# prstrive/SCGaussian

Measured on AMD Instinct MI355X. Metric: train_iters_per_sec, higher is better.
Workload: dtype f32; 1 GPU; S2: 200000 Gaussians, 1008x756, SH degree 3, fwd+bwd per view (BASELINE configs[1] shape: LLFF-fern 3-view training, 200 k Gaussians @ 1008x756); gaussians=200000, width=1008, height=756, sh_degree=3, visible=174771, views=3, parallelism=single, ranks_seen=1, launched_by=single process, grad_bucket_bytes=0, grad_bucket_bytes_per_view=0

## Files before the change

scgaussian_amd/csrc/blend.hip:

```cpp
#include "scg_common.h"
#include "tile_sort.h"

namespace scg {

constexpr float kHalfLog2e = 0.72134752044448170f;
typedef float f32x2 __attribute__((ext_vector_type(2)));
typedef float f32x4 __attribute__((ext_vector_type(4)));

__device__ __forceinline__ bool splat_hits_rect(const float4& a, const float4& b, float x0, float y0) {
    const float dx0 = x0 - a.x, dy0 = y0 - a.y, dx1 = dx0 + 7.0f, dy1 = dy0 + 7.0f;
    const float nx = __builtin_amdgcn_fmed3f(0.0f, dx0, dx1), ny = __builtin_amdgcn_fmed3f(0.0f, dy0, dy1);
    const float cb2 = a.w + a.w;
    const float ya = __builtin_amdgcn_fmed3f(b.w * nx, dy0, dy1);
    const float qa = nx * (a.z * nx + cb2 * ya) + b.x * ya * ya;
    const float xb = __builtin_amdgcn_fmed3f(-a.w * ny * __builtin_amdgcn_rcpf(a.z), dx0, dx1);
    const float qb = ny * (b.x * ny + cb2 * xb) + a.z * xb * xb;
    return !((qa > b.z) && (qb > b.z));
}

__device__ __forceinline__ int quadrant_workgroup(int wg, int n_tiles, const uint2* __restrict__ ranges, int& quad) {
    quad = (wg >> 3) & 3;
    const int per = (n_tiles + 7) >> 3;
    const uint32_t* order = reinterpret_cast<const uint32_t*>(ranges) + 2 * (size_t)n_tiles;
    return (int)order[(wg & 7) * per + (wg >> 5)];
}

__device__ __forceinline__ void wave_sync() {
    __builtin_amdgcn_fence(__ATOMIC_ACQ_REL, "wavefront");
    __builtin_amdgcn_wave_barrier();
}

typedef const uint32_t __attribute__((address_space(3))) * LdsIds;
template <class IdList>
__device__ __forceinline__ void forward_walk(float4* s_rec, const FrameDev& f, int tile, int quad, int lane, uint2 range,
                                             IdList list,
                                             const float4* __restrict__ splats, float* __restrict__ out_color,
                                             float* __restrict__ out_depth, float* __restrict__ out_alpha,
                                             float* __restrict__ final_T, uint32_t* __restrict__ n_contrib) {
    const int tile_x = tile % f.gx, tile_y = tile / f.gx;
    const int qx0 = tile_x * kTile + (quad & 1) * 8, qy0 = tile_y * kTile + (quad >> 1) * 8;
    const int px = qx0 + (lane & 7), py = qy0 + (lane >> 3);
    const bool inside = (px < f.W) && (py < f.H);
    const float pxf = (float)px, pyf = (float)py;

    const int n = (int)(range.y - range.x);
    float T = inside ? 1.0f : -1.0f;
    int bgi0 = __builtin_amdgcn_readfirstlane(__builtin_bit_cast(int, f.bg[0]));
    int bgi1 = __builtin_amdgcn_readfirstlane(__builtin_bit_cast(int, f.bg[1]));
    int bgi2 = __builtin_amdgcn_readfirstlane(__builtin_bit_cast(int, f.bg[2]));
    asm volatile("" : "+s"(bgi0), "+s"(bgi1), "+s"(bgi2));
    f32x2 Crg = {0.f, 0.f}, Cbz = {0.f, 0.f};
    uint32_t last = 0;
    int n_blended = 0;
#ifndef SCG_FWD_TRIP_CXX
    const uint32_t lds_base = (uint32_t)reinterpret_cast<uintptr_t>(s_rec);
    const uint64_t exec_all = __builtin_amdgcn_read_exec();
#endif

    uint32_t id_next = 0;
    float4 ra, rb, rc;
    if (n > 0) {
        const uint32_t id0 = list[min(lane, n - 1)];
        id_next = list[min(kWave + lane, n - 1)];
        ra = splats[3 * (size_t)id0 + 0]; rb = splats[3 * (size_t)id0 + 1]; rc = splats[3 * (size_t)id0 + 2];
    }

    for (int base = 0; base < n; base += kWave) {
        if (__all(T < 0.0f)) break;
        const bool hit = (base + lane < n) && splat_hits_rect(ra, rb, (float)qx0, (float)qy0);
        if (hit) {
            *reinterpret_cast<float2*>(&s_rec[2 * kWave + lane]) = make_float2(ra.x, ra.y);
            s_rec[kWave + lane] = make_float4(kHalfLog2e * ra.z, 2.0f * kHalfLog2e * ra.w, kHalfLog2e * rb.x, rb.y);
            s_rec[lane] = rc;
        }
        uint64_t m = __ballot(hit);
        if (base + kWave < n) {
            ra = splats[3 * (size_t)id_next + 0]; rb = splats[3 * (size_t)id_next + 1];
            rc = splats[3 * (size_t)id_next + 2];
            id_next = list[min(base + 2 * kWave + lane, n - 1)];
        }
        wave_sync();

        n_blended += __builtin_popcountll(m);
#ifdef SCG_FWD_TRIP_CXX
        while (m) {
            const int j = __builtin_ctzll(m);
            asm("s_bitset0_b64 %0, %1" : "+s"(m) : "s"(j));
            const float2 c = *reinterpret_cast<const float2*>(&s_rec[2 * kWave + j]);
            const float4 q = s_rec[kWave + j];
            const float dx = c.x - pxf, dy = c.y - pyf;
            const float u = __builtin_fmaf(q.y, dy, q.x * dx);
            const float t = __builtin_fmaf(u, dx, (q.z * dy) * dy);
            const float alpha = fminf(kAlphaMax, q.w * __builtin_amdgcn_exp2f(-t));
            const float wgt = T * alpha;
            const float test_T = __builtin_fmaf(-T, alpha, T);
            if ((t >= 0.0f) && (alpha >= kAlphaMin)) {
                const bool contributes = test_T >= kTEps;
                const float T_prev = T;
                T = contributes ? test_T : -fabsf(T_prev);
                if (contributes) {
                    const float4 col = s_rec[j];
                    const f32x2 ww = {wgt, wgt};
                    Crg = __builtin_elementwise_fma((f32x2){col.x, col.y}, ww, Crg);
                    Cbz = __builtin_elementwise_fma((f32x2){col.z, col.w}, ww, Cbz);
                    last = (uint32_t)(base + j + 1);
                }
            }
        }
#else
        int last_j = -1;
        while (m) {
            const int j = __builtin_ctzll(m);
            asm("s_bitset0_b64 %0, %1" : "+s"(m) : "s"(j));
            asm volatile(
                "v_lshl_add_u32 v63, %[j], 4, %[lds]\n\t"
                "ds_read_b64 v[48:49], v63 offset:2048\n\t"
                "ds_read_b128 v[52:55], v63 offset:1024\n\t"
                "s_waitcnt lgkmcnt(1)\n\t"
                "v_sub_f32_e32 v48, v48, %[px]\n\t"
                "v_sub_f32_e32 v49, v49, %[py]\n\t"
                "s_waitcnt lgkmcnt(0)\n\t"
                "v_mul_f32_e32 v58, v52, v48\n\t"
                "v_mul_f32_e32 v59, v54, v49\n\t"
                "v_fmac_f32_e32 v58, v53, v49\n\t"
                "v_mul_f32_e32 v60, v59, v49\n\t"
                "v_fmac_f32_e32 v60, v58, v48\n\t"
                "v_exp_f32_e64 v56, -v60\n\t"
                "v_cmpx_le_f32_e32 vcc, 0, v60\n\t"
                "v_mul_f32_e32 v56, v55, v56\n\t"
                "v_min_f32_e32 v56, 0x3f7d70a4, v56\n\t"
                "v_cmpx_le_f32_e32 vcc, %[amin], v56\n\t"
                "v_fma_f32 v57, -%[T], v56, %[T]\n\t"
                "v_mul_f32_e32 v56, %[T], v56\n\t"
                "v_or_b32_e32 %[T], 0x80000000, %[T]\n\t"
                "v_cmpx_le_f32_e32 vcc, %[eps], v57\n\t"
                "v_mov_b32_e32 %[T], v57\n\t"
                "ds_read_b128 v[44:47], v63\n\t"
                "v_mov_b32_e32 %[lj], %[j]\n\t"
                "s_waitcnt lgkmcnt(0)\n\t"
                "v_pk_fma_f32 %[crg], v[44:45], v[56:57], %[crg] op_sel_hi:[1,0,1]\n\t"
                "v_pk_fma_f32 %[cbz], v[46:47], v[56:57], %[cbz] op_sel_hi:[1,0,1]\n\t"
                "s_mov_b64 exec, %[all]"
                : [T] "+v"(T), [crg] "+v"(Crg), [cbz] "+v"(Cbz), [lj] "+v"(last_j)
                : [j] "s"(j), [lds] "v"(lds_base), [px] "v"(pxf), [py] "v"(pyf), [amin] "s"(kAlphaMin), [eps] "s"(kTEps),
                  [all] "s"(exec_all)
                : "memory", "vcc", "v44", "v45", "v46", "v47", "v48", "v49", "v52", "v53", "v54", "v55", "v56", "v57", "v58",
                  "v59", "v60", "v63");
        }
        if (last_j >= 0) last = (uint32_t)(base + last_j + 1);
#endif
        wave_sync();
    }

    if (f.cost_out && lane == 0) atomicMax(f.cost_out + tile, (uint32_t)n_blended);
    if (inside) {
        T = fabsf(T);
        const size_t pix = (size_t)py * f.W + px;
        const size_t hw = (size_t)f.H * f.W;
        out_color[pix] = Crg[0] + T * __builtin_bit_cast(float, bgi0);
        out_color[hw + pix] = Crg[1] + T * __builtin_bit_cast(float, bgi1);
        out_color[2 * hw + pix] = Cbz[0] + T * __builtin_bit_cast(float, bgi2);
        out_depth[pix] = Cbz[1];
        out_alpha[pix] = 1.0f - T;
        if (final_T) final_T[pix] = T;
        if (n_contrib) n_contrib[pix] = last;
    }
}


__global__ __launch_bounds__(kWave) void blend_forward_kernel(FrameDev f, const uint2* __restrict__ ranges,
                                                              const uint32_t* __restrict__ point_list,
                                                              const float4* __restrict__ splats,
                                                              float* __restrict__ out_color,
                                                              float* __restrict__ out_depth,
                                                              float* __restrict__ out_alpha,
                                                              float* __restrict__ final_T,
                                                              uint32_t* __restrict__ n_contrib,
                                                              float4* __restrict__ zero_fill, uint32_t zero_vec) {
    __shared__ float4 s_rec[3 * kWave];
    if (zero_fill) {
        for (uint32_t i = blockIdx.x * kWave + threadIdx.x; i < zero_vec; i += gridDim.x * kWave)
            zero_fill[i] = make_float4(0.f, 0.f, 0.f, 0.f);
    }

    const int n_tiles = f.gx * f.gy;
    int quad;
    const int tile = quadrant_workgroup(blockIdx.x, n_tiles, ranges, quad);
    if (tile >= n_tiles) return;
    const uint2 range = ranges[tile];
    forward_walk(s_rec, f, tile, quad, (int)threadIdx.x, range, point_list + range.x, splats, out_color, out_depth, out_alpha,
                 final_T, n_contrib);
}

template <int NW>
__device__ __forceinline__ void fused_long_list_fallback(unsigned char* smem, const uint32_t* __restrict__ depth_keys,
                                                      uint32_t* __restrict__ list, int n, uint64_t* __restrict__ keys,
                                                      uint64_t* __restrict__ keys2) {
    if (!sort_long_list<NW * kWave, kFusedLongBuckets, 2>(smem, depth_keys, list, n, keys, keys2)) {
        __syncthreads();
        for (int i = threadIdx.x; i < n; i += NW * kWave) {
            const uint32_t id = list[i];
            keys[i] = ((uint64_t)depth_keys[id] << 32) | (uint64_t)id;
        }
        __syncthreads();
        bitonic_sort_asc(keys, n, true);
        __syncthreads();
        for (int i = threadIdx.x; i < n; i += NW * kWave) list[i] = (uint32_t)keys[i];
    }
}

template <int MAX_N, int CNT, int WPE, int NW = 4>
__global__ __launch_bounds__(NW * kWave) __attribute__((amdgpu_waves_per_eu(WPE, WPE))) void tile_blend_forward_kernel(
    FrameDev f, const uint2* __restrict__ ranges, uint32_t* __restrict__ point_list,
    const uint32_t* __restrict__ depth_keys, int id_bits, const float4* __restrict__ splats,
    float* __restrict__ out_color, float* __restrict__ out_depth, float* __restrict__ out_alpha,
    float* __restrict__ final_T, uint32_t* __restrict__ n_contrib, float4* __restrict__ zero_fill, uint32_t zero_vec,
    uint64_t* __restrict__ spill, uint64_t* __restrict__ spill2, const uint32_t* __restrict__ class_counts,
    int long_presorted) {
    typedef TileSortLds<NW, MAX_N, CNT> Lds;
    constexpr size_t kIdsBytes = sizeof(uint32_t) * MAX_N, kPlanesBytes = 4 * 3 * kWave * sizeof(float4);
    constexpr size_t kLdsBytes = sizeof(Lds) > kIdsBytes + kPlanesBytes ? sizeof(Lds) : kIdsBytes + kPlanesBytes;
    __shared__ __attribute__((aligned(16))) unsigned char smem[kLdsBytes];
    Lds& L = *reinterpret_cast<Lds*>(smem);
    static_assert(offsetof(Lds, id) == 0, "the sorted ids lie in front of the record planes");
    static_assert(kLdsBytes >= (2 * kFusedLongBuckets + 4 + 2 * 4) * sizeof(uint32_t), "the fallback's counters must fit");
    if (zero_fill) {
        for (uint32_t i = blockIdx.x * blockDim.x + threadIdx.x; i < zero_vec; i += gridDim.x * blockDim.x)
            zero_fill[i] = make_float4(0.f, 0.f, 0.f, 0.f);
    }
    if (f.long_out && blockIdx.x == 0 && threadIdx.x == 0) {
        f.long_out[0] = class_counts[0] + class_counts[1];
        f.long_out[1] = class_counts[3];
    }
    const int n_tiles = f.gx * f.gy, per = (n_tiles + 7) >> 3;
    const uint32_t* order = reinterpret_cast<const uint32_t*>(ranges) + 2 * (size_t)n_tiles;
    const int tile = (int)order[(blockIdx.x & 7) * per + (blockIdx.x >> 3)];
    if (tile >= n_tiles) return;
    const uint2 range = ranges[tile];
    const int n = (int)(range.y - range.x);
#ifdef SCG_PROBE_TIMELINE
    const uint32_t tp0 = (uint32_t)wall_clock64();
#endif
    const bool ids_in_lds = n >= 2 && n <= MAX_N;
    if (ids_in_lds) sort_one_tile<NW, MAX_N, CNT, true>(L, range, depth_keys, point_list, id_bits);
    else if (n > MAX_N && !long_presorted)
        fused_long_list_fallback<NW>(smem, depth_keys, point_list + range.x, n, spill + range.x, spill2 + range.x);
#ifdef SCG_PROBE_TIMELINE
    const uint32_t tp1 = (uint32_t)wall_clock64();
    uint32_t pr[6];
    for (int k = 0; k < 6; ++k) pr[k] = L.probe[k];
    __syncthreads();
#else
    if (!ids_in_lds) __syncthreads();
#endif
    const int quad = (int)threadIdx.x >> 6, lane = (int)threadIdx.x & (kWave - 1);
    if (NW > 4 && quad >= 4) return;
#ifdef SCG_PROBE_TIMELINE
    const uint32_t tp2 = (uint32_t)wall_clock64();
#endif
    float4* planes = reinterpret_cast<float4*>(smem + kIdsBytes) + quad * 3 * kWave;
    if (ids_in_lds)
        forward_walk(planes, f, tile, quad, lane, range, reinterpret_cast<LdsIds>((uintptr_t)(uint32_t)reinterpret_cast<uintptr_t>(&L.id[0])),
                     splats, out_color, out_depth, out_alpha, final_T, n_contrib);
    else
        forward_walk(planes, f, tile, quad, lane, range, point_list + range.x, splats, out_color, out_depth, out_alpha, final_T,
                     n_contrib);
#ifdef SCG_PROBE_TIMELINE
    if (f.cost_out && lane == 0) {
        uint32_t* tl = f.cost_out + n_tiles + 65792 + 32768 + ((size_t)blockIdx.x * 4 + quad) * 8;
        tl[0] = tp0; tl[1] = tp1; tl[2] = tp2; tl[3] = (uint32_t)wall_clock64(); tl[4] = (uint32_t)n; tl[5] = (uint32_t)tile;
        tl[6] = 0u; tl[7] = 0xB1E9D000u;
        if (quad == 0) {
            uint32_t* t2 = f.cost_out + n_tiles + 65792 + 32768 + ((size_t)tile_order_slots(n_tiles) * 4 + blockIdx.x) * 8;
            for (int k = 0; k < 6; ++k) t2[k] = pr[k];
            t2[6] = tp0; t2[7] = 0x50B70000u;
        }
    }
#endif
}

int launch_tile_blend_forward(const FrameDev& f, const uint32_t* ranges, uint32_t* point_list, const uint32_t* depth_keys,
                              const float* splats, float* out_color, float* out_depth, float* out_alpha,
                              float* final_T, uint32_t* n_contrib, float* dsplats_zero, void* bin_scratch, int64_t R,
                              bool long_presorted, hipStream_t stream) {
    const int n_tiles = f.gx * f.gy;
    int id_bits = 8;
    while (id_bits < 32 && (1ll << id_bits) < (long long)f.P) id_bits += 8;
    const TileBinningLayout BL = tile_binning_layout(f.P, R, n_tiles);
    uint64_t* spill = reinterpret_cast<uint64_t*>(reinterpret_cast<char*>(bin_scratch) + BL.spill);
    const bool dense = fused_max_list(R, n_tiles) == kFusedDenseMaxN;
    auto kernel = dense ? tile_blend_forward_kernel<kFusedDenseMaxN, kFusedDenseCounters, kFusedDenseWpe, kFusedDenseWaves>
                        : tile_blend_forward_kernel<kFusedMaxN, kFusedCounters, 8>;
    hipLaunchKernelGGL(kernel, dim3(tile_order_slots(n_tiles)), dim3((dense ? kFusedDenseWaves : 4) * kWave), 0, stream, f,
                       reinterpret_cast<const uint2*>(ranges), point_list, depth_keys, id_bits,
                       reinterpret_cast<const float4*>(splats), out_color, out_depth, out_alpha, final_T, n_contrib,
                       reinterpret_cast<float4*>(dsplats_zero), (uint32_t)((size_t)f.P * SCG_DSPLAT_FLOATS / 4),
                       spill, spill + R,
                       reinterpret_cast<const uint32_t*>(reinterpret_cast<char*>(bin_scratch) + BL.class_counts),
                       long_presorted ? 1 : 0);
    return check_hip(hipGetLastError(), "tile_blend_forward_kernel");
}

int launch_blend_forward(const FrameDev& f, const uint32_t* ranges, const uint32_t* point_list,
                         const float* splats, float* out_color, float* out_depth, float* out_alpha,
                         float* final_T, uint32_t* n_contrib, float* dsplats_zero, hipStream_t stream) {
    const int n_tiles = f.gx * f.gy;
    const int grid = ((n_tiles + 7) / 8) * 8 * 4;
    hipLaunchKernelGGL(blend_forward_kernel, dim3(grid), dim3(kWave), 0, stream, f,
                       reinterpret_cast<const uint2*>(ranges), point_list, reinterpret_cast<const float4*>(splats),
                       out_color, out_depth, out_alpha, final_T, n_contrib, reinterpret_cast<float4*>(dsplats_zero),
                       (uint32_t)((size_t)f.P * SCG_DSPLAT_FLOATS / 4));
    return check_hip(hipGetLastError(), "blend_forward_kernel");
}


constexpr int kSlots = 4;
constexpr int kWStride = 2 * kWave;

__device__ __forceinline__ float row_reduce10(float v0, float v1, float v2, float v3, float v4, float v5, float v6,
                                              float v7, float v8, float v9, uint64_t odd, uint64_t hi) {
    float y, t0, t1, t2, t3, t4, t5, t6, t7;
    asm("s_nop 1\n\t"
        "v_add_f32_dpp %1, %9, %9 row_shl:4 row_mask:0xf bank_mask:0x5\n\t"
        "v_add_f32_dpp %2, %11, %11 row_shl:4 row_mask:0xf bank_mask:0x5\n\t"
        "v_add_f32_dpp %3, %13, %13 row_shl:4 row_mask:0xf bank_mask:0x5\n\t"
        "v_add_f32_dpp %4, %15, %15 row_shl:4 row_mask:0xf bank_mask:0x5\n\t"
        "v_add_f32_dpp %5, %17, %17 row_shl:4 row_mask:0xf bank_mask:0x5\n\t"
        "v_add_f32_dpp %1, %10, %10 row_shr:4 row_mask:0xf bank_mask:0xa\n\t"
        "v_add_f32_dpp %2, %12, %12 row_shr:4 row_mask:0xf bank_mask:0xa\n\t"
        "v_add_f32_dpp %3, %14, %14 row_shr:4 row_mask:0xf bank_mask:0xa\n\t"
        "v_add_f32_dpp %4, %16, %16 row_shr:4 row_mask:0xf bank_mask:0xa\n\t"
        "v_add_f32_dpp %5, %18, %18 row_shr:4 row_mask:0xf bank_mask:0xa\n\t"
        "v_add_f32_dpp %6, %1, %1 row_ror:8 row_mask:0xf bank_mask:0x3\n\t"
        "v_add_f32_dpp %7, %3, %3 row_ror:8 row_mask:0xf bank_mask:0x3\n\t"
        "v_add_f32_dpp %6, %2, %2 row_ror:8 row_mask:0xf bank_mask:0xc\n\t"
        "v_add_f32_dpp %7, %4, %4 row_ror:8 row_mask:0xf bank_mask:0xc\n\t"
        "v_add_f32_dpp %8, %5, %5 row_ror:8 row_mask:0xf bank_mask:0xf\n\t"
        "v_cndmask_b32 %1, %6, %7, %19\n\t"
        "v_cndmask_b32 %2, %7, %6, %19\n\t"
        "v_add_f32_dpp %3, %8, %8 quad_perm:[1,0,3,2] row_mask:0xf bank_mask:0xf\n\t"
        "s_nop 0\n\t"
        "v_add_f32_dpp %4, %2, %1 quad_perm:[1,0,3,2] row_mask:0xf bank_mask:0xf\n\t"
        "v_cndmask_b32 %5, %4, %3, %20\n\t"
        "v_cndmask_b32 %1, %3, %4, %20\n\t"
        "s_nop 1\n\t"
        "v_add_f32_dpp %0, %1, %5 quad_perm:[2,3,0,1] row_mask:0xf bank_mask:0xf"
        : "=&v"(y), "=&v"(t0), "=&v"(t1), "=&v"(t2), "=&v"(t3), "=&v"(t4), "=&v"(t5), "=&v"(t6), "=&v"(t7)
        : "v"(v0), "v"(v1), "v"(v2), "v"(v3), "v"(v4), "v"(v5), "v"(v6), "v"(v7), "v"(v8), "v"(v9), "s"(odd), "s"(hi));
    return y;
}

struct BwdLds {
    float4 a[kWave];
    float4 b[kWave];
    float4 c[kWave];
    __attribute__((aligned(16))) float w[kSlots * kWStride];
};

struct BwdPixel {
    float T, behind, dC0, dC1, dC2, dD, dA;
    uint32_t last;
};

__device__ __forceinline__ uint32_t top_chunk_index(int end) {
    return (uint32_t)min(((end - 1) / kWave) * kWave + (kWave - 1 - (int)threadIdx.x), end - 1);
}
__device__ __forceinline__ int backward_walk(BwdLds& L, const FrameDev& f, int tile, int quad, int first, int end,
                                              BwdPixel px, uint32_t list_begin, uint32_t id_top,
                                              const uint32_t* __restrict__ point_list,
                                              const float4* __restrict__ splats, float* __restrict__ dsplats) {
    const int lane = threadIdx.x;
    const int tile_x = tile % f.gx, tile_y = tile / f.gx;
    const int qx0 = tile_x * kTile + (quad & 1) * 8, qy0 = tile_y * kTile + (quad >> 1) * 8;
    const float pxf = (float)(qx0 + (lane & 7)), pyf = (float)(qy0 + (lane >> 3));
    float T = px.T, behind = px.behind;
    const float dC0 = px.dC0, dC1 = px.dC1, dC2 = px.dC2, dD = px.dD, dA = px.dA;
    const uint32_t last = px.last;

    const int row = lane >> 4, grp = lane & 15;
    float4 fc[4];
    {
        float4* tmp = reinterpret_cast<float4*>(L.w);
        __syncthreads();
        tmp[lane] = make_float4(dC0, dC1, dC2, dD);
        __syncthreads();
#pragma unroll
        for (int i = 0; i < 4; ++i) fc[i] = tmp[grp + 16 * i];
        __syncthreads();
    }
    const float gx_pix = (float)(qx0 + (grp & 7)), gy_pix = (float)(qy0 + (grp >> 3));
    float* w_store = L.w + 2 * lane;
#ifdef SCG_FWD_TRIP_CXX
    const float* w_load = L.w + row * kWStride + 2 * grp;
#else
    const uint32_t lds_wl = (uint32_t)reinterpret_cast<uintptr_t>(L.w + row * kWStride + 2 * grp);
    typedef const float __attribute__((address_space(3))) * LdsFloats;
#define w_load reinterpret_cast<LdsFloats>((uintptr_t)lds_wl)
#endif
    const int bank = (lane >> 2) & 3, qq_ = lane & 3;
    int out_slot = -1;
    if (qq_ < 2 || (qq_ == 2 && bank < 2)) {
        const int quantity = (qq_ == 0) ? bank : (qq_ == 1) ? 4 + bank : 8 + bank;
        out_slot = (quantity < 7) ? quantity : quantity + 1;
    }
    const uint32_t out_bytes = (uint32_t)(out_slot < 0 ? 0 : out_slot) * 4u;

    int slot = 0;
    float my_x = 0.f, my_y = 0.f;
    uint32_t my_id = 0;

    const uint64_t out_lanes = __ballot(out_slot >= 0);
    const uint64_t lanes_all = __builtin_amdgcn_read_exec();
    uint64_t odd_lanes = 0xAAAAAAAAAAAAAAAAull, hi_lanes = 0xCCCCCCCCCCCCCCCCull;
    asm volatile("" : "+s"(odd_lanes), "+s"(hi_lanes));
    auto flush = [&](int rows, float dx, float dy0) {
        __builtin_amdgcn_fence(__ATOMIC_ACQ_REL, "wavefront");
        __builtin_amdgcn_wave_barrier();
#ifdef SCG_FWD_TRIP_CXX
        const float2 qw0 = *reinterpret_cast<const float2*>(w_load);
#else
        const float2 qw0 = make_float2(w_load[0], w_load[1]);
#endif
        const float qy0 = qw0.x * dy0;
        float Sq = qw0.x, Sy = qy0, Syy = qy0 * dy0, Rr = qw0.y * fc[0].x, Gg = qw0.y * fc[0].y, Bb = qw0.y * fc[0].z,
              Dz = qw0.y * fc[0].w;
#pragma unroll
        for (int i = 1; i < 4; ++i) {
#ifdef SCG_FWD_TRIP_CXX
            const float2 qw = *reinterpret_cast<const float2*>(w_load + 32 * i);
#else
            const float2 qw = make_float2(w_load[32 * i], w_load[32 * i + 1]);
#endif
            const float dy = dy0 - (float)(2 * i);
            const float qy = qw.x * dy;
            Sq += qw.x;
            Sy += qy;
            Syy = __builtin_fmaf(qy, dy, Syy);
            Rr = __builtin_fmaf(qw.y, fc[i].x, Rr);
            Gg = __builtin_fmaf(qw.y, fc[i].y, Gg);
            Bb = __builtin_fmaf(qw.y, fc[i].z, Bb);
            Dz = __builtin_fmaf(qw.y, fc[i].w, Dz);
        }
        const float Sx = dx * Sq, Sxx = dx * Sx, Sxy = dx * Sy;
        const float sum = row_reduce10(Sx, Sy, Dz, Sq,
                                       Sxx, Sxy, Syy, Rr,
                                       Gg, Bb, odd_lanes, hi_lanes);
        const uint32_t rec = my_id * (uint32_t)(SCG_DSPLAT_FLOATS * 4) + out_bytes;
        const uint64_t lanes = (rows >= kSlots) ? out_lanes : (out_lanes & ((1ull << (16 * rows)) - 1ull));
        asm volatile("s_mov_b64 exec, %[lanes]\n\t"
                     "global_atomic_add_f32 %[off], %[val], %[base]\n\t"
                     "s_mov_b64 exec, %[all]"
                     :: [lanes] "s"(lanes), [off] "v"(rec), [val] "v"(sum), [base] "s"(dsplats), [all] "s"(lanes_all)
                     : "memory");
        __builtin_amdgcn_fence(__ATOMIC_ACQ_REL, "wavefront");
        __builtin_amdgcn_wave_barrier();
    };

    float amax_s;
    asm volatile("s_mov_b32 %0, 0x3f7d70a4" : "=s"(amax_s));
    const int chunk_bot = first / kWave;
    uint32_t id = id_top;
    int n_trips = 0;
#ifdef SCG_FWD_TRIP_CXX
    float* w_ptr = w_store;
#else
    static_assert(offsetof(BwdLds, b) == 1024 && offsetof(BwdLds, c) == 2048 && kWStride * sizeof(float) == 512,
                  "the hand-written walk addresses the planes with immediate offsets");
    const uint32_t lds_rec = (uint32_t)reinterpret_cast<uintptr_t>(&L.a[0]);
    const uint32_t lds_w = (uint32_t)reinterpret_cast<uintptr_t>(w_store);
    const uint64_t row0 = 0x000000000000FFFFull, row1 = 0x00000000FFFF0000ull, row2 = 0x0000FFFF00000000ull,
                   row3 = 0xFFFF000000000000ull;
    typedef float f32x16 __attribute__((ext_vector_type(16)));
    const f32x16 fcv = {fc[0].x, fc[0].y, fc[0].z, fc[0].w, fc[1].x, fc[1].y, fc[1].z, fc[1].w,
                        fc[2].x, fc[2].y, fc[2].z, fc[2].w, fc[3].x, fc[3].y, fc[3].z, fc[3].w};
    const f32x4 dCv = {dC0, dC1, dC2, dD};
#endif
    for (int chunk = (end - 1) / kWave; chunk >= chunk_bot; --chunk) {
        const int base = chunk * kWave;
        const int k = base + (kWave - 1 - lane);
#ifdef SCG_FWD_TRIP_CXX
        const int first_j = base + (kWave - 1) - (int)last;
#else
        const int first_j = max(base + (kWave - 1) - (int)last, -1);
#endif
        const float4 a = splats[3 * (size_t)id + 0];
        const float4 b = splats[3 * (size_t)id + 1];
        const float4 c_rec = splats[3 * (size_t)id + 2];
        uint32_t id_next = id;
        if (chunk > chunk_bot) id_next = point_list[list_begin + (uint32_t)(k - kWave)];
        const bool hit = (k < end) && splat_hits_rect(a, b, (float)qx0, (float)qy0);
        if (hit) {
            L.a[lane] = make_float4(a.x, a.y, kHalfLog2e * a.z, 2.0f * kHalfLog2e * a.w);
            L.b[lane] = make_float4(kHalfLog2e * b.x, b.y, __builtin_bit_cast(float, id), 0.f);
            L.c[lane] = c_rec;
        }
        id = id_next;
        uint64_t m = __ballot(hit);
        n_trips += __builtin_popcountll(m);
        __builtin_amdgcn_s_waitcnt(0x0F70);
        __syncthreads();

#ifdef SCG_FWD_TRIP_CXX
        while (m) {
            const int j = __builtin_ctzll(m);
            asm("s_bitset0_b64 %0, %1" : "+s"(m) : "s"(j));
            const float4 a = L.a[j];
            const float4 b = L.b[j];
            const float4 c = L.c[j];
            asm("" ::"v"(b.w));
            const float dx = a.x - pxf, dy = a.y - pyf;
            float u = a.z * dx;
            asm("" : "+v"(u));
            u = __builtin_fmaf(a.w, dy, u);
            const float t = __builtin_fmaf(u, dx, (b.x * dy) * dy);
            const float oG = b.y * __builtin_amdgcn_exp2f(-t);
            const bool ok = (j > first_j) && (t >= 0.0f) && (oG >= kAlphaMin);
            if (__ballot(ok) == 0ull) continue;

            const float q0 = ok ? oG : 0.0f;
            const float alpha = __builtin_amdgcn_fmed3f(q0, 0.0f, amax_s);
            const float one_m = 1.0f - alpha;
            T *= __builtin_amdgcn_rcpf(one_m);
            const float d = __builtin_fmaf(c.x, dC0, __builtin_fmaf(c.y, dC1, __builtin_fmaf(c.z, dC2, __builtin_fmaf(c.w, dD, dA))));
            const float q = q0 * ((d - behind) * T);
            behind *= one_m;
            asm("" : "+v"(behind));
            behind = __builtin_fmaf(alpha, d, behind);
            const float wgt = alpha * T;
            *reinterpret_cast<float2*>(w_ptr) = make_float2(q, wgt);
            w_ptr += kWStride;
            const bool mine = (row == slot);
            my_x = mine ? a.x : my_x;
            my_y = mine ? a.y : my_y;
            my_id = mine ? __builtin_bit_cast(uint32_t, b.z) : my_id;
            if (++slot == kSlots) {
                flush(kSlots, my_x - gx_pix, my_y - gy_pix);
                slot = 0;
                w_ptr = w_store;
            }
        }
#else
#define SCG_BWD_ROW(K, NEXT)                                                                                                 \
            ".Ltrip" #K "_%=:\n\t"                                                                                         \
            "s_ff1_i32_b64 s90, %[m]\n\t"                           \
            "s_bitset0_b64 %[m], s90\n\t"                                                                                 \
            "v_lshl_add_u32 v60, s90, 4, %[rec]\n\t"                                                                      \
            "ds_read_b128 v[48:51], v60\n\t"                                                                               \
            "ds_read_b128 v[52:55], v60 offset:1024\n\t"                                                                   \
            "ds_read_b128 v[44:47], v60 offset:2048\n\t"                                                                   \
            "v_mov_b32_e32 v58, 0\n\t"                                                                                     \
            "v_mov_b32_e32 v59, 0\n\t"                                                                                     \
            "v_cmpx_gt_i32_e32 vcc, s90, %[fj]\n\t"                 \
            "s_waitcnt lgkmcnt(2)\n\t"                                                                                     \
            "v_sub_f32_e32 v56, v48, %[px]\n\t"                                                                            \
            "v_sub_f32_e32 v57, v49, %[py]\n\t"                                                                            \
            "v_mul_f32_e32 v50, v56, v50\n\t"                                                                  \
            "s_waitcnt lgkmcnt(1)\n\t"                                                                                     \
            "v_mul_f32_e32 v52, v57, v52\n\t"                                                                  \
            "v_fmac_f32_e32 v50, v51, v57\n\t"                                                  \
            "v_mul_f32_e32 v52, v57, v52\n\t"                                                                \
            "v_fmac_f32_e32 v52, v50, v56\n\t"                                                            \
            "v_exp_f32_e64 v51, -v52\n\t"                                                                                  \
            "v_cmpx_le_f32_e32 vcc, 0, v52\n\t"                                                  \
            "v_mul_f32_e32 v51, v53, v51\n\t"                                                               \
            "v_cmpx_le_f32_e32 vcc, 0x3b808081, v51\n\t"                                \
            "s_cbranch_execz .Lnone" #K "_%=\n\t"                                                                          \
            "v_min_f32_e32 v50, 0x3f7d70a4, v51\n\t"                                     \
            "v_sub_f32_e32 v52, 1.0, v50\n\t"                                                       \
            "v_rcp_f32_e32 v56, v52\n\t"                                                                                   \
            "s_waitcnt lgkmcnt(0)\n\t"                                                                                     \
            "v_fma_f32 v57, v47, v27, %[dA]\n\t"                   \
            "v_fmac_f32_e32 v57, v46, v26\n\t"                                                                          \
            "v_fmac_f32_e32 v57, v45, v25\n\t"                                                                          \
            "v_fmac_f32_e32 v57, v44, v24\n\t"                                                                          \
            "v_mul_f32_e32 %[T], %[T], v56\n\t"                                  \
            "v_sub_f32_e32 v58, v57, %[bh]\n\t"                                                                            \
            "v_mul_f32_e32 v58, v58, %[T]\n\t"                                                                             \
            "v_mul_f32_e32 v58, v51, v58\n\t"                                                 \
            "v_mul_f32_e32 %[bh], %[bh], v52\n\t"                               \
            "v_fmac_f32_e32 %[bh], v50, v57\n\t"                                                                           \
            "v_mul_f32_e32 v59, v50, %[T]\n\t"                                                            \
            "s_mov_b64 exec, %[row" #K "]\n\t"                               \
            "v_sub_f32_e32 %[mdx], v48, %[px]\n\t"                     \
            "v_sub_f32_e32 %[mdy], v49, %[gy]\n\t"                                                                        \
            "v_mov_b32_e32 %[mi], v54\n\t"                                                                                 \
            "s_mov_b64 exec, -1\n\t"                                          \
            "ds_write_b64 %[wst], v[58:59] offset:" NEXT "\n\t"
#define SCG_BWD_NONE(K)                                                                                                      \
            ".Lnone" #K "_%=:\n\t"                                                                                         \
            "s_mov_b64 exec, -1\n\t"                                                                                   \
            "s_cmp_lt_i32 s90, 0\n\t"                                                                                     \
            "s_cbranch_scc0 .Ltrip" #K "_%=\n\t"                                                                           \
            "s_mov_b32 %[slot], " #K "\n\t"                                                                                \
            "s_branch .Lend_%=\n\t"
        {
            asm volatile(
                "s_cmp_eq_u32 %[slot], 0\n\t"
                "s_cbranch_scc1 .Ltrip0_%=\n\t"
                "s_cmp_eq_u32 %[slot], 1\n\t"
                "s_cbranch_scc1 .Ltrip1_%=\n\t"
                "s_cmp_eq_u32 %[slot], 2\n\t"
                "s_cbranch_scc1 .Ltrip2_%=\n\t"
                "s_branch .Ltrip3_%=\n\t"
                SCG_BWD_NONE(0)
                SCG_BWD_NONE(1)
                SCG_BWD_NONE(2)
                SCG_BWD_NONE(3)
                SCG_BWD_ROW(0, "0")
                SCG_BWD_ROW(1, "512")
                SCG_BWD_ROW(2, "1024")
                SCG_BWD_ROW(3, "1536")
                "ds_read2_b64 v[44:47], %[wld] offset1:16\n\t"
                "ds_read2_b64 v[48:51], %[wld] offset0:32 offset1:48\n\t"
                "v_add_f32_e32 v52, -2.0, %[mdy]\n\t"
                "v_add_f32_e32 v53, -4.0, %[mdy]\n\t"
                "v_add_f32_e32 v54, 0xc0c00000, %[mdy]\n\t"
                "s_waitcnt lgkmcnt(1)\n\t"
                "v_mul_f32_e32 v55, v44, %[mdy]\n\t"
                "v_mul_f32_e32 v57, v45, v28\n\t"
                "v_mul_f32_e32 v58, v45, v29\n\t"
                "v_mul_f32_e32 v59, v45, v30\n\t"
                "v_mul_f32_e32 v60, v45, v31\n\t"
                "v_mul_f32_e32 v56, v55, %[mdy]\n\t"
                "v_mul_f32_e32 v61, v46, v52\n\t"
                "v_add_f32_e32 v44, v44, v46\n\t"
                "v_fmac_f32_e32 v57, v47, v32\n\t"
                "v_fmac_f32_e32 v58, v47, v33\n\t"
                "v_fmac_f32_e32 v59, v47, v34\n\t"
                "v_fmac_f32_e32 v60, v47, v35\n\t"
                "v_add_f32_e32 v55, v55, v61\n\t"
                "v_fmac_f32_e32 v56, v61, v52\n\t"
                "s_waitcnt lgkmcnt(0)\n\t"
                "v_mul_f32_e32 v61, v48, v53\n\t"
                "v_add_f32_e32 v44, v44, v48\n\t"
                "v_fmac_f32_e32 v57, v49, v36\n\t"
                "v_fmac_f32_e32 v58, v49, v37\n\t"
                "v_fmac_f32_e32 v59, v49, v38\n\t"
                "v_fmac_f32_e32 v60, v49, v39\n\t"
                "v_add_f32_e32 v55, v55, v61\n\t"
                "v_fmac_f32_e32 v56, v61, v53\n\t"
                "v_mul_f32_e32 v61, v50, v54\n\t"
                "v_add_f32_e32 v44, v44, v50\n\t"
                "v_fmac_f32_e32 v57, v51, v40\n\t"
                "v_fmac_f32_e32 v58, v51, v41\n\t"
                "v_fmac_f32_e32 v59, v51, v42\n\t"
                "v_fmac_f32_e32 v60, v51, v43\n\t"
                "v_add_f32_e32 v55, v55, v61\n\t"
                "v_fmac_f32_e32 v56, v61, v54\n\t"
                "v_mul_f32_e32 v45, %[mdx], v44\n\t"
                "v_mul_f32_e32 v47, %[mdx], v55\n\t"
                "v_mul_f32_e32 v46, %[mdx], v45\n\t"
                "s_nop 1\n\t"
                "v_add_f32_dpp v48, v45, v45 row_shl:4 row_mask:0xf bank_mask:0x5\n\t"
                "v_add_f32_dpp v49, v60, v60 row_shl:4 row_mask:0xf bank_mask:0x5\n\t"
                "v_add_f32_dpp v50, v46, v46 row_shl:4 row_mask:0xf bank_mask:0x5\n\t"
                "v_add_f32_dpp v51, v56, v56 row_shl:4 row_mask:0xf bank_mask:0x5\n\t"
                "v_add_f32_dpp v52, v58, v58 row_shl:4 row_mask:0xf bank_mask:0x5\n\t"
                "v_add_f32_dpp v48, v55, v55 row_shr:4 row_mask:0xf bank_mask:0xa\n\t"
                "v_add_f32_dpp v49, v44, v44 row_shr:4 row_mask:0xf bank_mask:0xa\n\t"
                "v_add_f32_dpp v50, v47, v47 row_shr:4 row_mask:0xf bank_mask:0xa\n\t"
                "v_add_f32_dpp v51, v57, v57 row_shr:4 row_mask:0xf bank_mask:0xa\n\t"
                "v_add_f32_dpp v52, v59, v59 row_shr:4 row_mask:0xf bank_mask:0xa\n\t"
                "v_add_f32_dpp v53, v48, v48 row_ror:8 row_mask:0xf bank_mask:0x3\n\t"
                "v_add_f32_dpp v54, v50, v50 row_ror:8 row_mask:0xf bank_mask:0x3\n\t"
                "v_add_f32_dpp v53, v49, v49 row_ror:8 row_mask:0xf bank_mask:0xc\n\t"
                "v_add_f32_dpp v54, v51, v51 row_ror:8 row_mask:0xf bank_mask:0xc\n\t"
                "v_add_f32_dpp v61, v52, v52 row_ror:8 row_mask:0xf bank_mask:0xf\n\t"
                "v_cndmask_b32_e64 v48, v53, v54, %[odd]\n\t"
                "v_cndmask_b32_e64 v49, v54, v53, %[odd]\n\t"
                "v_add_f32_dpp v50, v61, v61 quad_perm:[1,0,3,2] row_mask:0xf bank_mask:0xf\n\t"
                "s_nop 0\n\t"
                "v_add_f32_dpp v51, v49, v48 quad_perm:[1,0,3,2] row_mask:0xf bank_mask:0xf\n\t"
                "v_cndmask_b32_e64 v52, v51, v50, %[hi]\n\t"
                "v_cndmask_b32_e64 v48, v50, v51, %[hi]\n\t"
                "v_lshl_add_u32 v44, %[mi], 6, %[ob]\n\t"
                "s_nop 0\n\t"
                "v_add_f32_dpp v45, v48, v52 quad_perm:[2,3,0,1] row_mask:0xf bank_mask:0xf\n\t"
                "s_mov_b64 exec, %[lanes]\n\t"
                "global_atomic_add_f32 v44, v45, %[base]\n\t"
                "s_mov_b64 exec, -1\n\t"
                "s_branch .Ltrip0_%=\n\t"
                ".Lend_%=:\n\t"
                "s_waitcnt lgkmcnt(0)"
                : [m] "+s"(m), [slot] "+s"(slot), [T] "+v"(T), [bh] "+v"(behind), [mdx] "+v"(my_x), [mdy] "+v"(my_y),
                  [mi] "+v"(my_id)
                : [rec] "v"(lds_rec), [wst] "v"(lds_w), [wld] "v"(lds_wl), [fj] "v"(first_j), [px] "v"(pxf), [py] "v"(pyf),
                  [gy] "v"(gy_pix), [ob] "v"(out_bytes), [dA] "v"(dA), "{v[24:27]}"(dCv), "{v[28:43]}"(fcv),
                  [row0] "s"(row0), [row1] "s"(row1), [row2] "s"(row2), [row3] "s"(row3), [lanes] "s"(out_lanes),
                  [odd] "s"(odd_lanes), [hi] "s"(hi_lanes), [base] "s"(dsplats)
                : "memory", "vcc", "scc", "s90", "s91", "v44", "v45", "v46", "v47", "v48", "v49", "v50", "v51", "v52", "v53",
                  "v54", "v55", "v56", "v57", "v58", "v59", "v60", "v61");
        }
#undef SCG_BWD_NONE
#undef SCG_BWD_ROW
#endif
        __syncthreads();
    }
#ifdef SCG_FWD_TRIP_CXX
    if (slot > 0) flush(slot, my_x - gx_pix, my_y - gy_pix);
#else
    if (slot > 0) flush(slot, my_x, my_y);
#undef w_load
#endif
    return n_trips;
}

__device__ __forceinline__ BwdPixel load_pixel_final(const FrameDev& f, int px, int py, const float* __restrict__ final_T,
                                                     const uint32_t* __restrict__ n_contrib,
                                                     const float* __restrict__ dL_dcolor, const float* __restrict__ dL_ddepth,
                                                     const float* __restrict__ dL_dalpha) {
    BwdPixel s;
    s.T = 1.0f; s.dC0 = s.dC1 = s.dC2 = s.dD = s.dA = 0.f; s.last = 0;
    if ((px < f.W) && (py < f.H)) {
        const size_t pix = (size_t)py * f.W + px;
        const size_t hw = (size_t)f.H * f.W;
        s.T = final_T[pix];
        s.last = n_contrib[pix];
        s.dC0 = dL_dcolor[pix]; s.dC1 = dL_dcolor[hw + pix]; s.dC2 = dL_dcolor[2 * hw + pix];
        if (dL_ddepth) s.dD = dL_ddepth[pix];
        if (dL_dalpha) s.dA = dL_dalpha[pix];
    }
    s.behind = f.bg[0] * s.dC0 + f.bg[1] * s.dC1 + f.bg[2] * s.dC2;
    return s;
}

#ifdef SCG_BWD_WAVES
#define SCG_BWD_OCCUPANCY __attribute__((amdgpu_waves_per_eu(SCG_BWD_WAVES, SCG_BWD_WAVES)))
#else
#define SCG_BWD_OCCUPANCY
#endif
__global__ __launch_bounds__(kWave) SCG_BWD_OCCUPANCY void blend_backward_kernel(
    FrameDev f, const uint2* __restrict__ ranges, const uint32_t* __restrict__ point_list,
    const float4* __restrict__ splats, const float* __restrict__ final_T, const uint32_t* __restrict__ n_contrib,
    const float* __restrict__ dL_dcolor, const float* __restrict__ dL_ddepth, const float* __restrict__ dL_dalpha,
    float* __restrict__ dsplats) {
    __shared__ BwdLds L;
    const int n_tiles = f.gx * f.gy;
    const int slots = tile_order_slots(n_tiles);
    const uint32_t* order_q = reinterpret_cast<const uint32_t*>(ranges) + 2 * (size_t)n_tiles + slots;
    const uint32_t entry = order_q[(size_t)(blockIdx.x & 7) * (4 * (slots >> 3)) + (blockIdx.x >> 3)];
    const int tile = (int)(entry >> 2), quad = (int)(entry & 3u);
    if (tile >= n_tiles) return;
    const int lane = threadIdx.x;
    const int px = (tile % f.gx) * kTile + (quad & 1) * 8 + (lane & 7), py = (tile / f.gx) * kTile + (quad >> 1) * 8 + (lane >> 3);
    const uint2 range = ranges[tile];
    const int n = (int)(range.y - range.x);
    const BwdPixel s = load_pixel_final(f, px, py, final_T, n_contrib, dL_dcolor, dL_ddepth, dL_dalpha);
    uint32_t mx = s.last;
#pragma unroll
    for (int off = 32; off > 0; off >>= 1) mx = max(mx, (uint32_t)__shfl_down((int)mx, off, kWave));
    const int limit = min(n, __builtin_amdgcn_readfirstlane((int)mx));
#ifdef SCG_PROBE_TIMELINE
    const uint32_t tp0 = (uint32_t)wall_clock64();
#endif
    if (limit <= 0) {
        if (f.bcost_out && lane == 0) f.bcost_out[4 * tile + quad] = 0u;
        return;
    }
    const int trips = backward_walk(L, f, tile, quad, 0, limit, s, range.x, point_list[range.x + top_chunk_index(limit)],
                                    point_list, splats, dsplats);
    if (f.bcost_out && lane == 0) f.bcost_out[4 * tile + quad] = (uint32_t)trips;
#ifdef SCG_PROBE_TIMELINE
    if (f.cost_out && lane == 0) {
        uint32_t* tl = f.cost_out + n_tiles + 65792 + 32768 + (size_t)(n_tiles + 8) * 40 + (size_t)blockIdx.x * 4;
        tl[0] = tp0; tl[1] = (uint32_t)wall_clock64(); tl[2] = ((uint32_t)min(trips, 65535) << 16) | (uint32_t)min(limit, 65535);
        tl[3] = 0xBAC00000u | (uint32_t)(4 * tile + quad);
    }
#endif
}

int launch_blend_backward(const FrameDev& f, const uint32_t* ranges, const uint32_t* point_list,
                          const float* splats, const float* final_T, const uint32_t* n_contrib,
                          const float* dL_dcolor, const float* dL_ddepth, const float* dL_dalpha,
                          float* dsplats, bool dsplats_prezeroed, hipStream_t stream, hipEvent_t started, hipEvent_t done) {
    if (!dsplats_prezeroed) {
        const int rc = check_hip(hipMemsetAsync(dsplats, 0, (size_t)f.P * SCG_DSPLAT_FLOATS * sizeof(float), stream),
                                 "dsplats memset");
        if (rc) return rc;
    }
    const int n_tiles = f.gx * f.gy;
    const int grid = ((n_tiles + 7) / 8) * 8 * 4;
    if (started || done) {
        hipExtLaunchKernelGGL(blend_backward_kernel, dim3(grid), dim3(kWave), 0u, stream, started, done, 0u, f,
                              reinterpret_cast<const uint2*>(ranges), point_list, reinterpret_cast<const float4*>(splats),
                              final_T, n_contrib, dL_dcolor, dL_ddepth, dL_dalpha, dsplats);
    } else {
        hipLaunchKernelGGL(blend_backward_kernel, dim3(grid), dim3(kWave), 0, stream, f,
                           reinterpret_cast<const uint2*>(ranges), point_list, reinterpret_cast<const float4*>(splats),
                           final_T, n_contrib, dL_dcolor, dL_ddepth, dL_dalpha, dsplats);
    }
    return check_hip(hipGetLastError(), "blend_backward_kernel");
}

}
```

Before: 4280 iters/s.

## Compact hit splats into dense LDS slots and unroll the blend loop by four

Each lane that passes the rect test now writes its record to a compacted LDS slot computed with mbcnt, and also stores its original list index next to its xy. The per-batch blend then walks a dense count instead of scanning the ballot mask with ctz and bit clears. The inline-asm path is reworked into an unrolled-by-four loop with constant LDS offsets, and it recovers the last contributor from the stored index. This trims the scalar overhead of each iteration in the hot forward rasterizer. In exchange the LDS stores become scattered and the assembly grows more complex.

```diff
diff --git a/scgaussian_amd/csrc/blend.hip b/scgaussian_amd/csrc/blend.hip
--- a/scgaussian_amd/csrc/blend.hip
+++ b/scgaussian_amd/csrc/blend.hip
@@ -5,6 +5,7 @@
 
 constexpr float kHalfLog2e = 0.72134752044448170f;
 typedef float f32x2 __attribute__((ext_vector_type(2)));
+typedef float f32x3 __attribute__((ext_vector_type(3)));
 typedef float f32x4 __attribute__((ext_vector_type(4)));
 
 __device__ __forceinline__ bool splat_hits_rect(const float4& a, const float4& b, float x0, float y0) {
@@ -68,12 +69,14 @@
     for (int base = 0; base < n; base += kWave) {
         if (__all(T < 0.0f)) break;
         const bool hit = (base + lane < n) && splat_hits_rect(ra, rb, (float)qx0, (float)qy0);
+        const uint64_t m = __ballot(hit);
+        const int cnt = __builtin_popcountll(m);
         if (hit) {
-            *reinterpret_cast<float2*>(&s_rec[2 * kWave + lane]) = make_float2(ra.x, ra.y);
-            s_rec[kWave + lane] = make_float4(kHalfLog2e * ra.z, 2.0f * kHalfLog2e * ra.w, kHalfLog2e * rb.x, rb.y);
-            s_rec[lane] = rc;
+            const uint32_t slot = __builtin_amdgcn_mbcnt_hi((uint32_t)(m >> 32), __builtin_amdgcn_mbcnt_lo((uint32_t)m, 0u));
+            *reinterpret_cast<f32x3*>(&s_rec[2 * kWave + slot]) = (f32x3){ra.x, ra.y, __builtin_bit_cast(float, base + lane + 1)};
+            s_rec[kWave + slot] = make_float4(kHalfLog2e * ra.z, 2.0f * kHalfLog2e * ra.w, kHalfLog2e * rb.x, rb.y);
+            s_rec[slot] = rc;
         }
-        uint64_t m = __ballot(hit);
         if (base + kWave < n) {
             ra = splats[3 * (size_t)id_next + 0]; rb = splats[3 * (size_t)id_next + 1];
             rc = splats[3 * (size_t)id_next + 2];
@@ -81,11 +84,10 @@
         }
         wave_sync();
 
-        n_blended += __builtin_popcountll(m);
+        n_blended += cnt;
 #ifdef SCG_FWD_TRIP_CXX
-        while (m) {
-            const int j = __builtin_ctzll(m);
-            asm("s_bitset0_b64 %0, %1" : "+s"(m) : "s"(j));
+        int last_slot = -1;
+        for (int j = 0; j < cnt; ++j) {
             const float2 c = *reinterpret_cast<const float2*>(&s_rec[2 * kWave + j]);
             const float4 q = s_rec[kWave + j];
             const float dx = c.x - pxf, dy = c.y - pyf;
@@ -103,51 +105,75 @@
                     const f32x2 ww = {wgt, wgt};
                     Crg = __builtin_elementwise_fma((f32x2){col.x, col.y}, ww, Crg);
                     Cbz = __builtin_elementwise_fma((f32x2){col.z, col.w}, ww, Cbz);
-                    last = (uint32_t)(base + j + 1);
+                    last_slot = j;
                 }
             }
         }
-#else
-        int last_j = -1;
-        while (m) {
-            const int j = __builtin_ctzll(m);
-            asm("s_bitset0_b64 %0, %1" : "+s"(m) : "s"(j));
-            asm volatile(
-                "v_lshl_add_u32 v63, %[j], 4, %[lds]\n\t"
-                "ds_read_b64 v[48:49], v63 offset:2048\n\t"
-                "ds_read_b128 v[52:55], v63 offset:1024\n\t"
-                "s_waitcnt lgkmcnt(1)\n\t"
-                "v_sub_f32_e32 v48, v48, %[px]\n\t"
-                "v_sub_f32_e32 v49, v49, %[py]\n\t"
-                "s_waitcnt lgkmcnt(0)\n\t"
-                "v_mul_f32_e32 v58, v52, v48\n\t"
-                "v_mul_f32_e32 v59, v54, v49\n\t"
-                "v_fmac_f32_e32 v58, v53, v49\n\t"
-                "v_mul_f32_e32 v60, v59, v49\n\t"
-                "v_fmac_f32_e32 v60, v58, v48\n\t"
-                "v_exp_f32_e64 v56, -v60\n\t"
-                "v_cmpx_le_f32_e32 vcc, 0, v60\n\t"
-                "v_mul_f32_e32 v56, v55, v56\n\t"
-                "v_min_f32_e32 v56, 0x3f7d70a4, v56\n\t"
-                "v_cmpx_le_f32_e32 vcc, %[amin], v56\n\t"
-                "v_fma_f32 v57, -%[T], v56, %[T]\n\t"
-                "v_mul_f32_e32 v56, %[T], v56\n\t"
-                "v_or_b32_e32 %[T], 0x80000000, %[T]\n\t"
-                "v_cmpx_le_f32_e32 vcc, %[eps], v57\n\t"
-                "v_mov_b32_e32 %[T], v57\n\t"
-                "ds_read_b128 v[44:47], v63\n\t"
-                "v_mov_b32_e32 %[lj], %[j]\n\t"
-                "s_waitcnt lgkmcnt(0)\n\t"
-                "v_pk_fma_f32 %[crg], v[44:45], v[56:57], %[crg] op_sel_hi:[1,0,1]\n\t"
-                "v_pk_fma_f32 %[cbz], v[46:47], v[56:57], %[cbz] op_sel_hi:[1,0,1]\n\t"
-                "s_mov_b64 exec, %[all]"
-                : [T] "+v"(T), [crg] "+v"(Crg), [cbz] "+v"(Cbz), [lj] "+v"(last_j)
-                : [j] "s"(j), [lds] "v"(lds_base), [px] "v"(pxf), [py] "v"(pyf), [amin] "s"(kAlphaMin), [eps] "s"(kTEps),
-                  [all] "s"(exec_all)
-                : "memory", "vcc", "v44", "v45", "v46", "v47", "v48", "v49", "v52", "v53", "v54", "v55", "v56", "v57", "v58",
-                  "v59", "v60", "v63");
-        }
-        if (last_j >= 0) last = (uint32_t)(base + last_j + 1);
+        if (last_slot >= 0) last = __builtin_bit_cast(uint32_t, s_rec[2 * kWave + last_slot].z);
+#else
+#define SCG_FWD_TRIP(RGB, CONIC, XY, NOTE)                                                                                   \
+                "ds_read_b64 v[48:49], v63 offset:" XY "\n\t"                                                              \
+                "ds_read_b128 v[52:55], v63 offset:" CONIC "\n\t"                                                          \
+                "s_waitcnt lgkmcnt(1)\n\t"                                                                                 \
+                "v_sub_f32_e32 v48, v48, %[px]\n\t"                                                                        \
+                "v_sub_f32_e32 v49, v49, %[py]\n\t"                                                                        \
+                "s_waitcnt lgkmcnt(0)\n\t"                                                                                 \
+                "v_mul_f32_e32 v58, v52, v48\n\t"                                                              \
+                "v_mul_f32_e32 v59, v54, v49\n\t"                                                              \
+                "v_fmac_f32_e32 v58, v53, v49\n\t"                                                  \
+                "v_mul_f32_e32 v60, v59, v49\n\t"                                                            \
+                "v_fmac_f32_e32 v60, v58, v48\n\t"                    \
+                "v_exp_f32_e64 v56, -v60\n\t"                                                                              \
+                "v_cmpx_le_f32_e32 vcc, 0, v60\n\t"                                                      \
+                "v_mul_f32_e32 v56, v55, v56\n\t"                                                                          \
+                "v_min_f32_e32 v56, 0x3f7d70a4, v56\n\t"                                 \
+                "v_cmpx_le_f32_e32 vcc, %[amin], v56\n\t"                                \
+                "v_fma_f32 v57, -%[T], v56, %[T]\n\t"                                                   \
+                "v_mul_f32_e32 v56, %[T], v56\n\t"                                                   \
+                "v_or_b32_e32 %[T], 0x80000000, %[T]\n\t"               \
+                "v_cmpx_le_f32_e32 vcc, %[eps], v57\n\t"                          \
+                "v_mov_b32_e32 %[T], v57\n\t"                                              \
+                "ds_read_b128 v[44:47], v63 offset:" RGB "\n\t"                                                            \
+                "v_add_u32_e32 %[la], " NOTE ", v63\n\t"                                     \
+                "s_waitcnt lgkmcnt(0)\n\t"                                                                                 \
+                "v_pk_fma_f32 %[crg], v[44:45], v[56:57], %[crg] op_sel_hi:[1,0,1]\n\t"                                    \
+                "v_pk_fma_f32 %[cbz], v[46:47], v[56:57], %[cbz] op_sel_hi:[1,0,1]\n\t"                                    \
+                "s_mov_b64 exec, %[all]\n\t"
+        uint32_t last_at = lds_base;
+        int groups, rest;
+        asm volatile(
+            "v_mov_b32_e32 v63, %[lds]\n\t"
+            "s_lshr_b32 %[g], %[cnt], 2\n\t"
+            "s_and_b32 %[r], %[cnt], 3\n\t"
+            "s_sub_u32 %[g], %[g], 1\n\t"
+            "s_cbranch_scc1 .Lrest_%=\n\t"
+            ".Lgroup_%=:\n\t"
+            SCG_FWD_TRIP("0", "1024", "2048", "16")
+            SCG_FWD_TRIP("16", "1040", "2064", "32")
+            SCG_FWD_TRIP("32", "1056", "2080", "48")
+            SCG_FWD_TRIP("48", "1072", "2096", "64")
+            "v_add_u32_e32 v63, 64, v63\n\t"
+            "s_sub_u32 %[g], %[g], 1\n\t"
+            "s_cbranch_scc0 .Lgroup_%=\n\t"
+            ".Lrest_%=:\n\t"
+            "s_sub_u32 %[r], %[r], 1\n\t"
+            "s_cbranch_scc1 .Ldone_%=\n\t"
+            ".Lone_%=:\n\t"
+            SCG_FWD_TRIP("0", "1024", "2048", "16")
+            "v_add_u32_e32 v63, 16, v63\n\t"
+            "s_sub_u32 %[r], %[r], 1\n\t"
+            "s_cbranch_scc0 .Lone_%=\n\t"
+            ".Ldone_%=:"
+            : [T] "+v"(T), [crg] "+v"(Crg), [cbz] "+v"(Cbz), [la] "+v"(last_at), [g] "=&s"(groups), [r] "=&s"(rest)
+            : [cnt] "s"(cnt), [lds] "v"(lds_base), [px] "v"(pxf), [py] "v"(pyf), [amin] "s"(kAlphaMin), [eps] "s"(kTEps),
+              [all] "s"(exec_all)
+            : "memory", "vcc", "scc", "v44", "v45", "v46", "v47", "v48", "v49", "v52", "v53", "v54", "v55", "v56", "v57", "v58",
+              "v59", "v60", "v63");
+#undef SCG_FWD_TRIP
+        static_assert(2 * kWave * sizeof(float4) + 8 - 16 == 2040, "the table word of slot s lies 2040 bytes behind its note");
+        typedef const uint32_t __attribute__((address_space(3))) * LdsWords;
+        const uint32_t noted = *reinterpret_cast<LdsWords>((uintptr_t)(last_at + 2040u));
+        last = (last_at != lds_base) ? noted : last;
 #endif
         wave_sync();
     }
```

Result: faster. 4338 iters/s, median of 6 (+1.4%).
